# bioinfologics/w2rap-contigger

Measured on AMD Instinct MI355X. Metric: step2_k60_canonical_kmers_per_s, higher is better.
Workload: dtype u64

## Files before the change

### include/w2rap_step2.h

```cpp
#ifndef W2RAP_STEP2_H_
#define W2RAP_STEP2_H_

#include <stddef.h>
#include <stdint.h>

#ifdef __cplusplus
extern "C" {
#endif

#define W2RAP_STEP2_ABI_VERSION 3

enum {
    W2RAP_OK = 0,
    W2RAP_E_ARG = 1,
    W2RAP_E_NO_DEVICE = 2,
    W2RAP_E_HIP = 3,
    W2RAP_E_STATE = 4,
    W2RAP_E_LIMIT = 5,
    W2RAP_E_GRAPH = 6,
    W2RAP_E_HINT = 7,
    W2RAP_E_IO = 8
};

enum { W2RAP_MEM_HOST = 0, W2RAP_MEM_DEVICE = 1 };
// ... 124 lines not shown
int w2rap_step2_solid_buffers(w2rap_step2_ctx*, void** d_hi, void** d_lo, void** d_cc, uint64_t* n);
int w2rap_step2_set_solid(w2rap_step2_ctx*, const void* d_hi, const void* d_lo, const void* d_cc, uint64_t n,
                          uint64_t M, uint64_t D, const uint64_t* hist101);
int w2rap_step2_chunk_buffers(w2rap_step2_ctx*, void** d_chunk_start, void** d_chunk_count, uint64_t* n_chunks);
int w2rap_step2_set_solid_chunked(w2rap_step2_ctx*, const void* d_hi, const void* d_lo, const void* d_cc, uint64_t n,
                                  uint64_t M, uint64_t D, const uint64_t* hist101,
                                  const void* d_chunk_start, const void* d_chunk_count, uint64_t n_chunks);

int w2rap_step2_dict_begin(w2rap_step2_ctx*, uint64_t kmer_capacity, uint64_t chunk_capacity);
int w2rap_step2_dict_append(w2rap_step2_ctx*, const void* d_hi, const void* d_lo, const void* d_cc, uint64_t n,
                            const void* d_chunk_start, const void* d_chunk_count, uint64_t n_chunks);
int w2rap_step2_dict_append_slice(w2rap_step2_ctx*, const void* d_hi, const void* d_lo, const void* d_cc, uint64_t n,
                                  const void* d_chunk_start, const void* d_chunk_count, uint64_t n_chunks, uint64_t chunk_bias);
int w2rap_step2_dict_end(w2rap_step2_ctx*, uint64_t M, uint64_t D, const uint64_t* hist101);
int w2rap_step2_dict_abort(w2rap_step2_ctx*);

enum { W2RAP_X_DONE = 0, W2RAP_X_ALLTOALL = 1, W2RAP_X_ALLGATHER = 2, W2RAP_X_ALLGATHER_HOST = 3, W2RAP_X_ALLREDUCE_U8 = 4, W2RAP_X_ALLREDUCE_U32 = 5 };
typedef struct w2rap_xchg {
    int32_t  op;
    uint32_t elem_bytes;
    void*    send;
    uint64_t send_count[64];
} w2rap_xchg;
int w2rap_step2_shard_begin(w2rap_step2_ctx*, uint32_t rank, uint32_t world, const uint64_t* solid_per_rank ,
                            uint32_t n_buckets, uint32_t n_passes, uint64_t M, uint64_t D, const uint64_t* hist101,
                            const w2rap_edge_hint* hint );
int w2rap_step2_local_dict_slice(w2rap_step2_ctx*, uint64_t n_solid, uint64_t expected_total);
int w2rap_step2_shard_next(w2rap_step2_ctx*, w2rap_xchg* x);
int w2rap_step2_shard_recv(w2rap_step2_ctx*, const uint64_t* recv_count , uint32_t elem_bytes, void** d_recv);
int w2rap_step2_shard_host_words(w2rap_step2_ctx*, const uint64_t* words );
int w2rap_step2_shard_info(w2rap_step2_ctx*, uint64_t out[8]);
int w2rap_step2_selftest_prims(w2rap_step2_ctx*, uint64_t n, uint64_t seed, int key_bits);
int w2rap_step2_selftest_filter32(w2rap_step2_ctx*, uint64_t nbases, uint64_t seed, uint32_t w_lo_frac16, uint32_t w_hi_frac16);
uint64_t w2rap_step2_device_bytes(w2rap_step2_ctx*);
uint64_t w2rap_step2_device_peak_bytes(w2rap_step2_ctx*, int reset);

#ifdef __cplusplus
}
#endif
#endif
```

### w2rap_contigger_amd/csrc/common.h

```cpp
#pragma once
#include <hip/hip_runtime.h>
#include <stdint.h>

namespace w2 {

constexpr unsigned K = 60;
constexpr unsigned MMER_F = 15;
constexpr uint64_t M60 = (1ull << 60) - 1;
constexpr uint64_t EMPTY_HI = ~0ull;
constexpr uint32_t NONE32 = 0xFFFFFFFFu;

struct Kmer { uint64_t hi, lo; };

__host__ __device__ inline uint64_t rev2_64(uint64_t x) {
#if defined(__HIP_DEVICE_COMPILE__)
    x = __brevll(x);
#else
    x = ((x >> 1) & 0x5555555555555555ull) | ((x & 0x5555555555555555ull) << 1);
    x = ((x >> 2) & 0x3333333333333333ull) | ((x & 0x3333333333333333ull) << 2);
    x = ((x >> 4) & 0x0F0F0F0F0F0F0F0Full) | ((x & 0x0F0F0F0F0F0F0F0Full) << 4);
    x = __builtin_bswap64(x);
#endif
    return ((x >> 1) & 0x5555555555555555ull) | ((x & 0x5555555555555555ull) << 1);
}
// ... 130 lines not shown
    const unsigned long long x = w[v + RT_NODES - (o & 0xFFFu)];
    end = (Id)RankW<Id>::next(x);
    dist = end == v ? 0u : (uint32_t)RankW<Id>::dist(x) - (o >> 12);
}
template <class Id, unsigned U, class T>
__device__ inline void rank_of_staged(const uint32_t* __restrict__ own, const unsigned long long* __restrict__ w, const T* __restrict__ at_end,
                                      const uint64_t (&i)[U], Id (&end)[2 * U], uint32_t (&dist)[2 * U], T (&end_val)[2 * U]) {
    uint32_t o[2 * U]; unsigned long long x[2 * U];
#pragma unroll
    for (unsigned j = 0; j < U; ++j) { const uint2 t = *reinterpret_cast<const uint2*>(&own[2 * i[j]]); o[2 * j] = t.x; o[2 * j + 1] = t.y; }
#pragma unroll
    for (unsigned n = 0; n < 2 * U; ++n) {
        const uint64_t v = 2 * i[n / 2] + (n & 1);
        x[n] = w[o[n] == OWN_CIRCLE ? v : v + RT_NODES - (o[n] & 0xFFFu)];
    }
#pragma unroll
    for (unsigned n = 0; n < 2 * U; ++n) {
        const Id v = (Id)(2 * i[n / 2] + (n & 1));
        end[n] = o[n] == OWN_CIRCLE ? v : (Id)RankW<Id>::next(x[n]);
        dist[n] = end[n] == v ? 0u : (uint32_t)RankW<Id>::dist(x[n]) - (o[n] >> 12);
    }
#pragma unroll
    for (unsigned n = 0; n < 2 * U; ++n) end_val[n] = at_end[end[n]];
}
template <class Id>
__device__ inline uint32_t edge_of_end(const unsigned long long* __restrict__ w, Id t) {
    return (uint32_t)RankW<Id>::dist(w[t]) - 1u;
}

struct alignas(32) ObjRec { int32_t succ[4]; uint32_t eo_lo, eo_hi, elen, edge_rc ; };

constexpr unsigned FMER = 31;
constexpr unsigned FSPAN = K - FMER;
struct FmerKey { uint32_t word; uint64_t mask; };
__host__ __device__ inline FmerKey fmer_key(uint64_t x) {
    x &= (1ull << (2 * FMER)) - 1;
    const uint64_t rx = rev2_64(~x) >> (64 - 2 * FMER);
    uint32_t mu = 0xFFFFFFFFu;
#pragma unroll
    for (unsigned j = 0; j <= FMER - MMER_F; j += 4) {
        const uint32_t f = (uint32_t)(x >> (2 * j)) & 0x3FFFFFFFu, r = (uint32_t)(rx >> (2 * (FMER - MMER_F - j))) & 0x3FFFFFFFu;
        const uint32_t key = (f < r ? f : r) * 0x9E3779B1u;
        mu = key < mu ? key : mu;
    }
    uint32_t w = mu ^ (mu >> 15); w *= 0x85EBCA6Bu; w ^= w >> 13;
    const uint64_t h = (rx < x ? rx : x) * 0x9E3779B97F4A7C15ull;
    return FmerKey{w, (1ull << ((h >> 58) & 63)) | (1ull << ((h >> 40) & 63))};
}

#ifndef W2RAP_REC36
constexpr unsigned REC_DWORDS = 8;
constexpr unsigned REC_MAXK = 63;
constexpr unsigned REC_HB = 8;
#else
constexpr unsigned REC_DWORDS = 9;
constexpr unsigned REC_MAXK = 64;
constexpr unsigned REC_HB = 32;
#endif
constexpr unsigned REC_BYTES = 4 * REC_DWORDS;

__host__ __device__ inline void rec_build(const uint8_t* __restrict__ bases, uint64_t bases_bytes, uint64_t ro, uint32_t meta, uint32_t (&out)[REC_DWORDS]) {
    const unsigned p = meta & 0xFFFFu, nk = ((meta >> 16) & 63u) + 1u;
    const bool hasL = (meta >> 22) & 1u, hasR = (meta >> 23) & 1u;
    const unsigned q = p ? p - 1 : 0;
    const uint64_t byte0 = ro + ((2 * q) >> 3);
    const unsigned sh = (2 * q) & 7;
    uint64_t W[5];
#pragma unroll
    for (unsigned j = 0; j < 5; ++j) {
        const uint64_t a = byte0 + 8 * j;
        uint64_t w = 0;
        if (a + 8 <= bases_bytes) w = reinterpret_cast<const U64u*>(bases + a)->v;
        else for (unsigned t = 0; t < 8; ++t) if (a + t < bases_bytes) w |= (uint64_t)bases[a + t] << (8 * t);
        W[j] = w;
    }
    uint64_t O[4];
#pragma unroll
    for (unsigned j = 0; j < 4; ++j) O[j] = sh ? (W[j] >> sh) | (W[j + 1] << (64 - sh)) : W[j];
    if (!p) {
        O[3] = (O[3] << 2) | (O[2] >> 62); O[2] = (O[2] << 2) | (O[1] >> 62); O[1] = (O[1] << 2) | (O[0] >> 62); O[0] <<= 2;
// ... 207 lines not shown
```

### w2rap_contigger_amd/csrc/step2_graph.hip

```cpp
#include <algorithm>
#include <cstring>
#include <vector>
#include "ctx.h"

namespace w2 {

enum { GE_LOOKUP = 1, GE_OFFSET = 2, GE_HINT_MISS = 4, GE_HINT_DUP = 8, GE_ASSIGN = 16, GE_HINT_LEN = 32 };

template <class Id>
__device__ inline Kmer oriented(const uint64_t* shi, const uint64_t* slo, Id v) {
    Kmer k{shi[v >> 1], slo[v >> 1]};
    return (v & 1) ? kmer_rc(k) : k;
}

template <class Id>
__global__ void __launch_bounds__(256) k_links(uint64_t S, const uint64_t* __restrict__ shi, const uint64_t* __restrict__ slo,
                                                const uint8_t* __restrict__ sctx, Id* nbr_nxt0) {
    constexpr Id NONE = NodeId<Id>::NONE, PAL = NodeId<Id>::PAL;
    uint64_t i = (uint64_t)blockIdx.x * blockDim.x + threadIdx.x;
    if (i >= S) return;
    Kmer k{shi[i], slo[i]};
    Id n0 = NONE, n1 = NONE;
    if (!kmer_is_pal(k)) {
        const Id s = nbr_nxt0[2 * i], p = nbr_nxt0[2 * i + 1];
// ... 468 lines not shown
        } else dst[K - 1 + off[j]] = (uint8_t)kmer_last(k);
    }
}
template <class Id>
__global__ void __launch_bounds__(256) k_assign(uint64_t S, const uint64_t* __restrict__ shi, const uint64_t* __restrict__ slo,
                                                 const uint32_t* __restrict__ own, const unsigned long long* __restrict__ w,
                                                 const uint64_t* __restrict__ edge_off, KRec* __restrict__ srec,
                                                 uint8_t* __restrict__ codes, uint32_t* __restrict__ flags) {
    if (((uint64_t)blockIdx.x + 1) * (256 * RANK_U) <= S) assign_block<Id, true>(S, shi, slo, own, w, edge_off, srec, codes, flags);
    else assign_block<Id, false>(S, shi, slo, own, w, edge_off, srec, codes, flags);
}

__global__ void __launch_bounds__(256) k_pack_codes(uint64_t nbytes, uint64_t nbases, const uint8_t* __restrict__ codes, uint8_t* __restrict__ bits) {
    uint64_t i = (uint64_t)blockIdx.x * blockDim.x + threadIdx.x;
    if (i >= nbytes) return;
    unsigned v = 0;
#pragma unroll
    for (unsigned j = 0; j < 4; ++j) { uint64_t g = 4 * i + j; if (g < nbases) v |= (unsigned)(codes[g] & 3) << (2 * j); }
    bits[i] = (uint8_t)v;
}

__global__ void __launch_bounds__(256) k_filter32(uint64_t npos, const uint8_t* __restrict__ bits, unsigned long long* __restrict__ filter,
                                                   uint32_t fmask, uint32_t w_lo, uint32_t w_hi) {
    const uint64_t g = (uint64_t)blockIdx.x * blockDim.x + threadIdx.x;
    const unsigned lane = threadIdx.x & 63;
    uint32_t word = 0xFFFFFFFFu; unsigned long long mask = 0;
    if (g < npos) {
        const uint64_t b0 = g >> 2; const unsigned sh = 2 * (unsigned)(g & 3);
        uint64_t x = reinterpret_cast<const U64u*>(bits + b0)->v >> sh;
        if (sh) x |= (uint64_t)bits[b0 + 8] << (64 - sh);
        const FmerKey k = fmer_key(x);
        word = k.word & fmask; mask = k.mask;
    }
    const uint32_t prev = __shfl_up(word, 4);
    const bool head = g < npos && (lane < 4 || prev != word);
#pragma unroll
    for (unsigned d = 4; d < 64; d <<= 1) {
        const uint32_t ow = __shfl_down(word, d);
        const unsigned long long om = __shfl_down(mask, d);
        if (lane + d < 64 && ow == word) mask |= om;
    }
    if (head && word - w_lo < w_hi - w_lo) atomicOr(&filter[word - w_lo], mask);
}

__global__ void __launch_bounds__(256) k_index_tails(uint64_t E, const uint64_t* __restrict__ edge_off, const uint32_t* __restrict__ edge_nk,
                                                      uint32_t* __restrict__ bad) {
    const uint64_t e = (uint64_t)blockIdx.x * blockDim.x + threadIdx.x;
    if (e >= E) return;
    const uint64_t g1 = edge_off[e] + edge_nk[e] + (K - 1), g0 = g1 - (MMER - 1);
    for (uint64_t wd = g0 >> 5; wd <= (g1 - 1) >> 5; ++wd) {
        const uint64_t lo = wd << 5;
        const unsigned a = g0 > lo ? (unsigned)(g0 - lo) : 0u, b = g1 - lo < 32 ? (unsigned)(g1 - lo) : 32u;
        const uint32_t m = (b == 32 ? 0xFFFFFFFFu : (1u << b) - 1u) & ~((1u << a) - 1u);
        atomicOr(&bad[wd], m);
    }
}
constexpr unsigned IS = 2048, IT = IS - (WIN - 1);
constexpr unsigned IT_EDGES = IT / K + 3;
__global__ void __launch_bounds__(256) k_index_tile_edge(uint64_t E, const uint64_t* __restrict__ edge_off, uint32_t* __restrict__ tile_edge) {
    const uint64_t e = (uint64_t)blockIdx.x * blockDim.x + threadIdx.x;
    if (e >= E) return;
    const uint64_t a = edge_off[e], b = edge_off[e + 1];
    for (uint64_t t = (a + IT - 1) / IT; t * IT < b; ++t) tile_edge[t] = (uint32_t)e;
}
template <int MODE>
__global__ void __launch_bounds__(256) k_index_build(uint64_t nbases, const uint8_t* __restrict__ ebits, const uint32_t* __restrict__ bad, uint64_t E,
                                                      const uint64_t* __restrict__ edge_off, const uint32_t* __restrict__ tile_edge,
                                                      uint4* __restrict__ slots, uint64_t mask, unsigned long long* __restrict__ counter, uint64_t blk0) {
    constexpr bool WRITE = MODE != 0;
    constexpr unsigned NKEY = IS + (WIN - 1) + 3;
// ... 191 lines not shown
    uint64_t j = (uint64_t)blockIdx.x * blockDim.x + threadIdx.x;
    if (j >= n) return;
    uint32_t f = 0;
    if (j > 0) {
        uint32_t a = perm[j - 1], b = perm[j];
        const bool same_seq = ehi[a] == ehi[b] && elo[a] == elo[b];
        f = (ehash[a] != ehash[b] || !same_seq) ? 1u : 0u;
        if (ehash[a] == ehash[b] && !same_seq) *shared_hash = 1u;
    }
    flag[j] = f;
}
__global__ void __launch_bounds__(256) k_tie_sort_lo(uint64_t E, const uint64_t* __restrict__ shi, const uint64_t* __restrict__ lo, uint32_t* __restrict__ perm,
                                                      unsigned max_run, uint32_t* __restrict__ long_run ) {
    const uint64_t j = (uint64_t)blockIdx.x * blockDim.x + threadIdx.x;
    if (j >= E || (j > 0 && shi[j] == shi[j - 1])) return;
    uint64_t b = j + 1;
    while (b < E && shi[b] == shi[j]) ++b;
    if (b - j > max_run) { *long_run = 1u; return; }
    for (uint64_t i = j + 1; i < b; ++i) {
        const uint32_t x = perm[i]; const uint64_t lx = lo[x];
        uint64_t t = i;
        while (t > j && lo[perm[t - 1]] > lx) { perm[t] = perm[t - 1]; --t; }
        perm[t] = x;
    }
}
__global__ void __launch_bounds__(256) k_end_vertices(uint64_t n, const uint32_t* __restrict__ perm, const uint32_t* __restrict__ flag,
                                                       const uint64_t* __restrict__ excl, int32_t* __restrict__ left, int32_t* __restrict__ right) {
    uint64_t j = (uint64_t)blockIdx.x * blockDim.x + threadIdx.x;
    if (j >= n) return;
    int32_t vid = (int32_t)(excl[j] + flag[j]);
    uint32_t id = perm[j];
    if (id & 1) right[id >> 1] = vid; else left[id >> 1] = vid;
}
__global__ void __launch_bounds__(256) k_adj_keys(uint64_t NO, const int32_t* __restrict__ a, const int32_t* __restrict__ b,
                                                   uint64_t* __restrict__ keys, uint32_t* __restrict__ vals, uint32_t* __restrict__ deg) {
    uint64_t o = (uint64_t)blockIdx.x * blockDim.x + threadIdx.x;
    if (o >= NO) return;
    keys[o] = ((uint64_t)(uint32_t)a[o] << 32) | (uint32_t)b[o];
    vals[o] = (uint32_t)o;
    atomicAdd(&deg[a[o]], 1u);
}
__global__ void __launch_bounds__(256) k_adj_out(uint64_t NO, const uint32_t* __restrict__ vals, const int32_t* __restrict__ other,
                                                  int32_t* __restrict__ out_v, int32_t* __restrict__ out_e) {
    uint64_t j = (uint64_t)blockIdx.x * blockDim.x + threadIdx.x;
    if (j >= NO) return;
    uint32_t o = vals[j];
    out_e[j] = (int32_t)o; out_v[j] = other[o];
}

__device__ inline unsigned obj_base(const uint8_t* codes, uint64_t eoff, uint32_t len, bool rc, uint32_t t);
__global__ void __launch_bounds__(256) k_obj_table(uint64_t NO, const uint32_t* __restrict__ obj_edge, const uint32_t* __restrict__ edge_nk,
                                                    const uint64_t* __restrict__ edge_off, const uint8_t* __restrict__ codes,
                                                    const int32_t* __restrict__ right, const uint64_t* __restrict__ from_off,
                                                    const int32_t* __restrict__ from_e, ObjRec* __restrict__ tab) {
    const uint64_t o = (uint64_t)blockIdx.x * blockDim.x + threadIdx.x;
    if (o >= NO) return;
    const uint32_t oe = obj_edge[o], e = oe >> 1;
    const uint64_t eo = edge_off[e];
    ObjRec r;
    r.succ[0] = r.succ[1] = r.succ[2] = r.succ[3] = -1;
    r.eo_lo = (uint32_t)eo; r.eo_hi = (uint32_t)(eo >> 32); r.elen = edge_nk[e] + (K - 1); r.edge_rc = oe;
    const int32_t v = right[o];
    for (uint64_t k = from_off[v]; k < from_off[v + 1]; ++k) {
        const int32_t o2 = from_e[k];
        const uint32_t oe2 = obj_edge[o2], e2 = oe2 >> 1, len2 = edge_nk[e2] + (K - 1);
        const unsigned b = obj_base(codes, edge_off[e2], len2, oe2 & 1, K - 1);
        r.succ[b] = o2;
    }
    tab[o] = r;
}

// ... 570 lines not shown
    if (NE) {
        LAUNCH(c, "k_ends", k_ends, dim3(grid_for(NE)), dim3(256), 0, NO, c.d_obj_edge, c.d_edge_off, c.d_edge_nk, c.d_edge_codes, ehash, ehi, elo);
        bool by_bases = test_hook("W2RAP_TEST_ENDS_FULL_SORT");
        uint64_t nflag = 0;
        for (;;) {
            LAUNCH(c, "k_iota", k_iota, dim3(grid_for(NE)), dim3(256), 0, NE, eperm);
            if (by_bases) {
                LAUNCH(c, "k_gather_u64", k_gather_u64, dim3(grid_for(NE)), dim3(256), 0, NE, elo, eperm, ktmp);
                W2_TRY(sort_pairs_u64(c, ktmp, eperm, NE, 0, 58));
                LAUNCH(c, "k_gather_u64", k_gather_u64, dim3(grid_for(NE)), dim3(256), 0, NE, ehi, eperm, ktmp);
                W2_TRY(sort_pairs_u64(c, ktmp, eperm, NE, 0, 60));
            }
            LAUNCH(c, "k_gather_u64", k_gather_u64, dim3(grid_for(NE)), dim3(256), 0, NE, ehash, eperm, ktmp);
            W2_TRY(sort_pairs_u64(c, ktmp, eperm, NE, 0, 64));
            W2_HIP(hipMemsetAsync(d_flags + 3, 0, 4, st));
            LAUNCH(c, "k_end_flags", k_end_flags, dim3(grid_for(NE)), dim3(256), 0, NE, eperm, ehash, ehi, elo, eflag, d_flags + 3);
            W2_TRY(exclusive_scan_u32_to_u64(c, eflag, excl, NE));
            uint32_t shared_hash = 0;
            W2_HIP(hipMemcpyAsync(&nflag, excl + NE, 8, hipMemcpyDeviceToHost, st));
            W2_HIP(hipMemcpyAsync(&shared_hash, d_flags + 3, 4, hipMemcpyDeviceToHost, st));
            W2_HIP(hipStreamSynchronize(st));
            if (shared_hash && !by_bases) { by_bases = true; continue; }
            break;
        }
        c.NV = nflag + 1;
        LAUNCH(c, "k_end_vertices", k_end_vertices, dim3(grid_for(NE)), dim3(256), 0, NE, eperm, eflag, excl, c.d_left, c.d_right);
    }
    const uint64_t NV = c.NV;
    W2_ALLOC(c.d_from_off, uint64_t, NV + 1); W2_ALLOC(c.d_to_off, uint64_t, NV + 1);
    W2_ALLOC(c.d_from_v, int32_t, NO); W2_ALLOC(c.d_from_e, int32_t, NO);
    W2_ALLOC(c.d_to_v, int32_t, NO); W2_ALLOC(c.d_to_e, int32_t, NO);
    uint32_t* deg = nullptr; uint64_t* akeys = nullptr; uint32_t* avals = nullptr;
    W2_ALLOC(deg, uint32_t, NV); W2_ALLOC(akeys, uint64_t, NO); W2_ALLOC(avals, uint32_t, NO);
    for (int dir = 0; dir < 2; ++dir) {
        const int32_t* a = dir == 0 ? c.d_left : c.d_right;
        const int32_t* b = dir == 0 ? c.d_right : c.d_left;
        W2_HIP(hipMemsetAsync(deg, 0, (NV ? NV : 1) * 4, st));
        if (NO) {
            LAUNCH(c, "k_adj_keys", k_adj_keys, dim3(grid_for(NO)), dim3(256), 0, NO, a, b, akeys, avals, deg);
            W2_TRY(sort_pairs_u64(c, akeys, avals, NO, 0, 64));
            LAUNCH(c, "k_adj_out", k_adj_out, dim3(grid_for(NO)), dim3(256), 0, NO, avals, b, dir == 0 ? c.d_from_v : c.d_to_v,
                               dir == 0 ? c.d_from_e : c.d_to_e);
        }
        W2_TRY(exclusive_scan_u32_to_u64(c, deg, dir == 0 ? c.d_from_off : c.d_to_off, NV));
    }
    if (c.d_otab) { c.release(c.d_otab); c.d_otab = nullptr; }
    W2_ALLOC(c.d_otab, ObjRec, NO);
    if (NO) LAUNCH(c, "k_obj_table", k_obj_table, dim3(grid_for(NO)), dim3(256), 0, NO, c.d_obj_edge, c.d_edge_nk, c.d_edge_off, c.d_edge_codes,
                   c.d_right, c.d_from_off, c.d_from_e, c.d_otab);
    W2_HIP(hipStreamSynchronize(st));
    if (c.stream2) W2_HIP(hipStreamSynchronize(c.stream2));
    W2_HIP(hipGetLastError());
    for (void* p : {(void*)d_nobj, (void*)d_ooff, (void*)ehash, (void*)ehi, (void*)elo, (void*)ktmp, (void*)excl,
                    (void*)eperm, (void*)eflag, (void*)deg, (void*)akeys, (void*)avals, (void*)d_flags})
        c.release(p);
    c.graphed = true;
    return 0;
}

template <class Id>
static int phase_graph_t(Ctx& c, const w2rap_edge_hint* hint) {
    constexpr Id NONE = NodeId<Id>::NONE; (void)NONE;
    hipStream_t st = c.stream;
    const uint64_t S = c.S, N = 2 * S;
    const uint64_t mask = c.tcap - 1;
    uint32_t* d_flags = nullptr;
    W2_ALLOC(d_flags, uint32_t, 8);
    W2_HIP(hipMemsetAsync(d_flags, 0, 32, st));
    Id* nxt0 = reinterpret_cast<Id*>(c.d_nbr);
    unsigned long long* rankw = nullptr; uint32_t* own = nullptr;
    W2_ALLOC(rankw, unsigned long long, N); W2_ALLOC(own, uint32_t, N);
    uint8_t *cyc = nullptr, *mid = nullptr, *is_head = nullptr;
    W2_ALLOC(cyc, uint8_t, N); W2_ALLOC(mid, uint8_t, N);
// ... 77 lines not shown
    c.release(is_head); is_head = nullptr;
    uint32_t* d_elen = nullptr;
    W2_ALLOC(d_elen, uint32_t, E);
    W2_ALLOC(c.d_edge_off, uint64_t, E + 1);
    if (E) LAUNCH(c, "k_edge_len", k_edge_len, dim3(grid_for(E)), dim3(256), 0, E, c.d_edge_nk, d_elen);
    W2_TRY(exclusive_scan_u32_to_u64(c, d_elen, c.d_edge_off, E));
    W2_HIP(hipMemcpyAsync(&c.edge_bases, c.d_edge_off + E, 8, hipMemcpyDeviceToHost, st));
    W2_HIP(hipStreamSynchronize(st));
    W2_ALLOC(c.d_edge_codes, uint8_t, c.edge_bases + 64);
    {
        const char* iv = getenv("W2RAP_PATH_INDEX");
        c.use_index = iv && atoi(iv) != 0;
    }
    if (c.d_srec) { c.release(c.d_srec); c.d_srec = nullptr; }
    if (!c.use_index) W2_ALLOC(c.d_srec, KRec, S);
    if (S) LAUNCH(c, "k_assign", k_assign<Id>, dim3(grid_per_thread(S, RANK_U)), dim3(256), 0, S, c.d_shi, c.d_slo, own, rankw,
                              c.d_edge_off, c.d_srec, c.d_edge_codes, d_flags);
    W2_HIP(hipStreamSynchronize(st));
    c.release(rankw); c.release(own); rankw = nullptr; own = nullptr;
    for (void* p : {(void*)d_nheads, (void*)head_v, (void*)perm, (void*)edge_head, (void*)key_hi, (void*)key_lo, (void*)key_tmp, (void*)d_elen, (void*)d_flags})
        c.release(p);
    return graph_finish(c);
}

int phase_graph(Ctx& c, const w2rap_edge_hint* hint) {
    if (!c.counted) { c.err = "build_graph called before count_kmers"; return W2RAP_E_STATE; }
    if (!c.d_nbr && c.S) { c.err = "build_graph: the neighbour links of this count have been consumed; call count_kmers again"; return W2RAP_E_STATE; }
    c.graphed = false;
    return c.wide_ids ? phase_graph_t<uint64_t>(c, hint) : phase_graph_t<uint32_t>(c, hint);
}

}

extern "C" int w2rap_step2_selftest_filter32(w2rap_step2_ctx* h, uint64_t nbases, uint64_t seed, uint32_t w_lo_frac16, uint32_t w_hi_frac16) {
    using namespace w2;
    if (!h || nbases < FMER || nbases > (1ull << 33) || w_lo_frac16 > w_hi_frac16 || w_hi_frac16 > 16) return -1;
    Ctx& c = h->c;
    if (hipSetDevice(c.device) != hipSuccess) return -1;
    const uint64_t nby = (nbases + 3) / 4;
    std::vector<uint8_t> hb(nby + 16, 0);
    uint64_t x = seed * 0x9E3779B97F4A7C15ull + 1;
    for (uint64_t g = 0; g < nbases; ++g) {
        x ^= x << 13; x ^= x >> 7; x ^= x << 17;
        hb[g >> 2] |= (uint8_t)(((x >> 33) & 3) << (2 * (g & 3)));
    }
    const uint64_t fw = filter32_words_for(nbases), lo = fw * w_lo_frac16 / 16, hi = fw * w_hi_frac16 / 16, npos = nbases - (FMER - 1);
    std::vector<unsigned long long> want(hi - lo + 1, 0), got(hi - lo + 1);
    for (uint64_t g = 0; g < npos; ++g) {
        const uint64_t b0 = g >> 2; const unsigned sh = 2 * (unsigned)(g & 3);
        uint64_t v; std::memcpy(&v, &hb[b0], 8);
        v >>= sh;
        if (sh) v |= (uint64_t)hb[b0 + 8] << (64 - sh);
        const FmerKey k = fmer_key(v);
        const uint64_t word = k.word & (uint32_t)(fw - 1);
        if (word >= lo && word < hi) want[word - lo] |= k.mask;
    }
    uint8_t* d_bits = c.alloc<uint8_t>(nby + 16, false);
    unsigned long long* d_out = c.alloc<unsigned long long>(hi - lo + 1, false);
    if (!d_bits || !d_out) return -1;
    int bad = 0;
    if (hipMemcpyAsync(d_bits, hb.data(), nby + 16, hipMemcpyHostToDevice, c.stream) != hipSuccess ||
        filter32_build(c, c.stream, d_bits, nbases, fw, lo, hi, d_out, hi - lo + 1) ||
        hipMemcpyAsync(got.data(), d_out, (hi - lo + 1) * 8, hipMemcpyDeviceToHost, c.stream) != hipSuccess ||
        hipStreamSynchronize(c.stream) != hipSuccess) bad = -1;
    for (uint64_t i = 0; i < hi - lo && !bad; ++i) if (got[i] != want[i]) bad = 1;
    if (!bad && got[hi - lo] != 0) bad = 2;
    c.release(d_bits); c.release(d_out);
    return bad;
}
```

### w2rap_contigger_amd/csrc/step2_path.hip

```cpp
#include <algorithm>
#include <cstdlib>
#include <type_traits>
#include "ctx.h"

namespace w2 {

#ifdef W2RAP_IDX_STATS
#define SITE_STAT(k) do { const unsigned long long am_ = __ballot(1); if ((threadIdx.x & 63) == (unsigned)__builtin_ctzll(am_)) { atomicAdd(&g_site_stats[2 * (k)], (unsigned long long)__builtin_popcountll(am_)); atomicAdd(&g_site_stats[2 * (k) + 1], 1ull); } } while (0)
static __device__ unsigned long long g_site_stats[8];
#else
#define SITE_STAT(k) ((void)0)
#endif
constexpr unsigned PCS = 256;
constexpr unsigned LP = 2;
constexpr unsigned PL = 4;
constexpr unsigned PATH_THREADS = 256;
constexpr uint32_t LONG_READ = 1024;
constexpr uint64_t SCRATCH_CAP = 16ull << 30;
constexpr uint64_t LONG_SCRATCH = 2ull << 30;
#ifndef W2RAP_PATH_TICKETS
#define W2RAP_PATH_TICKETS 1
#endif
constexpr uint32_t PATH_TICKETS = W2RAP_PATH_TICKETS;
struct PathArgs {
// ... 306 lines not shown
        const uint64_t bo = A.boff[live ? r : (LISTED ? r : r0)];
        bool deferred = false;
        uint32_t my_off = 0;
        if (STAGED) {
            const uint64_t b_lo = A.boff[r0], b_hi = A.boff[r0 + nr], a0 = b_lo & ~3ull;
            const uint32_t nbytes = (uint32_t)(b_hi - a0), nfull = nbytes >> 2;
            const uint32_t* src = reinterpret_cast<const uint32_t*>(A.bases + a0);
            for (uint32_t i = tid; i < nfull; i += PATH_THREADS) s_rd[i] = src[i];
            if (tid < 4) s_rd[nfull + 1 + tid] = 0;
            if (tid == 0) {
                uint32_t v = 0;
                for (uint32_t t2 = 0; t2 < (nbytes & 3); ++t2) v |= (uint32_t)A.bases[a0 + 4ull * nfull + t2] << (8 * t2);
                s_rd[nfull] = v;
            }
            my_off = (uint32_t)(bo - a0);
            __syncthreads();
        }
        uint32_t plen = 0, lo = A.pmid, hi = A.pmid;
        int32_t offset = 0;
        if (live) {
#ifdef W2RAP_IDX_STATS
            const unsigned long long ts0 = __builtin_amdgcn_s_memtime();
#endif
            const uint8_t* rb = A.bases + bo;
            const uint8_t* q = A.quals + A.qoff[r];
            const uint32_t L = A.len[r];
            uint32_t np = 0;
            typename std::conditional<STAGED, RdLds, RdGlb>::type rd;
            if constexpr (STAGED) { rd.w = s_rd; rd.off = my_off; } else { rd.rb = rb; rd.nby = (L + 3) >> 2; }
            if (L < K) { setp(0, make_gap(L)); np = 1; }
            else {
                uint32_t p = 0;
                const uint32_t end = L - K + 1;
                auto mer32_at = [&](uint32_t tt) -> FmerKey { return fmer_key(rd.bits64(tt)); };
                auto f32_absent = [&](const FmerKey& k, unsigned long long w) -> bool { return (w & k.mask) != k.mask; };
                const uint32_t last = L - K, tmax = L - FMER;
                auto probe3 = [&](uint32_t cur0, uint32_t e) -> uint32_t {
                    const uint32_t qmax = e < last ? e : last;
                    auto target = [&](uint32_t c_) -> uint32_t { uint32_t tt = c_ + FSPAN < e ? c_ + FSPAN : e; return tt > tmax ? tmax : tt; };
                    uint32_t cur = cur0;
                    const bool v0 = cur <= qmax; const uint32_t t0 = target(cur), q0 = t0 < last ? t0 : last; if (v0) cur = q0 + 1;
                    const bool v1 = v0 && cur <= qmax; const uint32_t t1 = target(cur), q1 = t1 < last ? t1 : last; if (v1) cur = q1 + 1;
                    const bool v2 = v1 && cur <= qmax; const uint32_t t2 = target(cur), q2 = t2 < last ? t2 : last;
                    FmerKey k0{0, 0}, k1{0, 0}, k2{0, 0}; unsigned long long w0 = 0, w1 = 0, w2 = 0;
                    if (v0) { k0 = mer32_at(t0); w0 = A.filter32[k0.word & A.f32mask]; }
                    if (v1) { k1 = mer32_at(t1); w1 = A.filter32[k1.word & A.f32mask]; }
                    if (v2) { k2 = mer32_at(t2); w2 = A.filter32[k2.word & A.f32mask]; }
                    const bool a0 = v0 && f32_absent(k0, w0), a1 = a0 && v1 && f32_absent(k1, w1), a2 = a1 && v2 && f32_absent(k2, w2);
                    return a2 ? q2 + 1 - cur0 : a1 ? q1 + 1 - cur0 : a0 ? q0 + 1 - cur0 : 0u;
                };
                bool mism = false;
                uint32_t pv_e = 0, pv_elen = 0, pv_i = 0, pv_j = 0; uint64_t pv_eo = 0; bool pv_rc = false;
                bool at_end = false;
                int32_t pv_obj = 0;
                while (p != end) {
                    if (!LISTED && A.part_budget && np >= A.part_budget) { deferred = true; break; }
                    bool hit = false; IdxHit ih{};
                    auto lookup = [&](uint32_t pp) -> bool { return dict_lookup<INDEX>(A, rd, pp, ih); };
                    uint32_t gapLen = 0;
                    bool probed = false;
                    const bool after_mism = mism;
                    if (mism && A.filter32) { gapLen = probe3(p, p + (K - 1)); p += gapLen; probed = gapLen != 0; }
                    mism = false;
                    bool diag_hit = false; uint32_t dg_off = 0;
                    bool ask_dict = !gapLen;
                    if (at_end) {
                        const unsigned nb_ = (unsigned)(rd.bits64(p + (K - 1)) & 3u);
// ... 175 lines not shown
            const unsigned want = (unsigned)__builtin_popcountll(free_m);
            const int leader = __builtin_ctzll(free_m);
            unsigned long long base = 0;
            if ((int)lane == leader) base = atomicAdd(&A.stripes[(size_t)stripe * STRIPE_PAD], (unsigned long long)want);
            base = __shfl(base, leader);
            const uint64_t s_lo = (uint64_t)stripe * per_stripe, s_hi = s_lo + per_stripe < n_all ? s_lo + per_stripe : n_all;
            const uint64_t idx = s_lo + base + (unsigned)__builtin_popcountll(free_m & ((1ull << lane) - 1));
            if (!has && !ready && idx < s_hi) {
                r = A.r_first + idx;
                const uint64_t bo = A.boff[r];
                L = A.len[r];
                const uint32_t nby = (L + 3) >> 2;
                for (uint32_t o = 0; o < A.slot_dwords * 4; o += 16) {
                    uint4 v = make_uint4(0, 0, 0, 0);
                    if (o < nby + 8) {
                        if (bo + o + 16 <= A.bases_bytes) { const U128u w = *reinterpret_cast<const U128u*>(A.bases + bo + o); v = make_uint4((uint32_t)w.a, (uint32_t)(w.a >> 32), (uint32_t)w.b, (uint32_t)(w.b >> 32)); }
                        else {
                            uint32_t t4[4] = {0, 0, 0, 0};
                            for (uint32_t t2 = 0; t2 < 16 && bo + o + t2 < A.bases_bytes; ++t2) t4[t2 >> 2] |= (uint32_t)A.bases[bo + o + t2] << (8 * (t2 & 3));
                            v = make_uint4(t4[0], t4[1], t4[2], t4[3]);
                        }
                    }
                    *reinterpret_cast<uint4*>(slot + (o >> 2)) = v;
                }
                has = true; deferred = false; np = 0; p = 0; mism = false; at_end = false;
                if (L < K) { setp(0, make_gap(L)); np = 1; end = 0; }
                else end = L - K + 1;
            }
            if (s_lo + base + want >= s_hi) { ++stripes_done; stripe = (stripe + 1) % NSTR; }
        }
        if (has && p != end) {
            if (A.part_budget && np >= A.part_budget) { deferred = true; p = end; }
            else {
                auto mer32_at = [&](uint32_t tt) -> FmerKey { return fmer_key(rd.bits64(tt)); };
                auto f32_absent = [&](const FmerKey& k, unsigned long long w) -> bool { return (w & k.mask) != k.mask; };
                const uint32_t last = L - K, tmax = L - FMER;
                auto probe3 = [&](uint32_t cur0, uint32_t e) -> uint32_t {
                    const uint32_t qmax = e < last ? e : last;
                    auto target = [&](uint32_t c_) -> uint32_t { uint32_t tt = c_ + FSPAN < e ? c_ + FSPAN : e; return tt > tmax ? tmax : tt; };
                    uint32_t cur = cur0;
                    const bool v0 = cur <= qmax; const uint32_t t0 = target(cur), q0 = t0 < last ? t0 : last; if (v0) cur = q0 + 1;
                    const bool v1 = v0 && cur <= qmax; const uint32_t t1 = target(cur), q1 = t1 < last ? t1 : last; if (v1) cur = q1 + 1;
                    const bool v2 = v1 && cur <= qmax; const uint32_t t2 = target(cur), q2 = t2 < last ? t2 : last;
                    FmerKey k0{0, 0}, k1{0, 0}, k2{0, 0}; unsigned long long w0 = 0, w1 = 0, w2 = 0;
                    if (v0) { k0 = mer32_at(t0); w0 = A.filter32[k0.word & A.f32mask]; }
                    if (v1) { k1 = mer32_at(t1); w1 = A.filter32[k1.word & A.f32mask]; }
                    if (v2) { k2 = mer32_at(t2); w2 = A.filter32[k2.word & A.f32mask]; }
                    const bool a0 = v0 && f32_absent(k0, w0), a1 = a0 && v1 && f32_absent(k1, w1), a2 = a1 && v2 && f32_absent(k2, w2);
                    return a2 ? q2 + 1 - cur0 : a1 ? q1 + 1 - cur0 : a0 ? q0 + 1 - cur0 : 0u;
                };
                bool hit = false; IdxHit ih{};
                auto lookup = [&](uint32_t pp) -> bool { return dict_lookup<INDEX>(A, rd, pp, ih); };
                uint32_t gapLen = 0;
                bool probed = false;
                const bool after_mism = mism;
                if (mism && A.filter32) { gapLen = probe3(p, p + (K - 1)); p += gapLen; probed = gapLen != 0; }
                mism = false;
                bool diag_hit = false; uint32_t dg_off = 0;
                bool ask_dict = !gapLen;
                if (at_end) {
                    const unsigned nb_ = (unsigned)(rd.bits64(p + (K - 1)) & 3u);
                    const int32_t o2 = A.otab[pv_obj].succ[nb_];
                    if (o2 >= 0) {
                        const ObjRec r2 = A.otab[o2];
                        diag_hit = true; dg_off = 0; ask_dict = false;
                        pv_e = r2.edge_rc >> 1; pv_rc = r2.edge_rc & 1u; pv_elen = r2.elen; pv_eo = (uint64_t)r2.eo_lo | ((uint64_t)r2.eo_hi << 32);
                    }
// ... 617 lines not shown
```

Measured before the change: 44.91 billion.

## Sample filter minimizers at stride two and narrow adjacency sort keys

The 31-mer filter key now takes the minimizer over window offsets at stride 2 instead of 4. This gives denser minimizer sampling, so more equal filter words are shared between neighbouring positions and the path-stage filter probes should give fewer false hits, at the cost of more hashing work per key and scheduling barriers in the path kernels. The gather shuffle distance follows the new stride. Separately, adjacency sort keys pack vertex ids into only as many bits as needed, so the radix sort runs over fewer key bits. A periodic-sequence self-test for the filter is added.

```diff
diff --git a/include/w2rap_step2.h b/include/w2rap_step2.h
--- a/include/w2rap_step2.h
+++ b/include/w2rap_step2.h
@@ -180,6 +180,7 @@
 int w2rap_step2_shard_info(w2rap_step2_ctx*, uint64_t out[8]);
 int w2rap_step2_selftest_prims(w2rap_step2_ctx*, uint64_t n, uint64_t seed, int key_bits);
 int w2rap_step2_selftest_filter32(w2rap_step2_ctx*, uint64_t nbases, uint64_t seed, uint32_t w_lo_frac16, uint32_t w_hi_frac16);
+int w2rap_step2_selftest_filter32_periodic(w2rap_step2_ctx*, uint64_t nbases, uint32_t period, uint64_t seed, uint32_t w_lo_frac16, uint32_t w_hi_frac16);
 uint64_t w2rap_step2_device_bytes(w2rap_step2_ctx*);
 uint64_t w2rap_step2_device_peak_bytes(w2rap_step2_ctx*, int reset);
 
diff --git a/w2rap_contigger_amd/csrc/common.h b/w2rap_contigger_amd/csrc/common.h
--- a/w2rap_contigger_amd/csrc/common.h
+++ b/w2rap_contigger_amd/csrc/common.h
@@ -186,20 +186,34 @@
 
 constexpr unsigned FMER = 31;
 constexpr unsigned FSPAN = K - FMER;
+#ifndef W2RAP_FMER_STRIDE
+#define W2RAP_FMER_STRIDE 2
+#endif
+constexpr unsigned FMER_STRIDE = W2RAP_FMER_STRIDE;
+static_assert(FMER_STRIDE >= 1 && (FMER - MMER_F) % FMER_STRIDE == 0, "the window offsets must map onto themselves under j <-> 16 - j");
 struct FmerKey { uint32_t word; uint64_t mask; };
+template <unsigned STRIDE = FMER_STRIDE, bool FENCED = false>
 __host__ __device__ inline FmerKey fmer_key(uint64_t x) {
+    static_assert(STRIDE >= 1 && (FMER - MMER_F) % STRIDE == 0, "stride must divide 16");
     x &= (1ull << (2 * FMER)) - 1;
     const uint64_t rx = rev2_64(~x) >> (64 - 2 * FMER);
     uint32_t mu = 0xFFFFFFFFu;
-#pragma unroll
-    for (unsigned j = 0; j <= FMER - MMER_F; j += 4) {
+#if defined(__HIP_DEVICE_COMPILE__)
+    if (FENCED) __builtin_amdgcn_sched_barrier(0);
+#endif
+#pragma unroll
+    for (unsigned j = 0; j <= FMER - MMER_F; j += STRIDE) {
         const uint32_t f = (uint32_t)(x >> (2 * j)) & 0x3FFFFFFFu, r = (uint32_t)(rx >> (2 * (FMER - MMER_F - j))) & 0x3FFFFFFFu;
         const uint32_t key = (f < r ? f : r) * 0x9E3779B1u;
         mu = key < mu ? key : mu;
     }
     uint32_t w = mu ^ (mu >> 15); w *= 0x85EBCA6Bu; w ^= w >> 13;
     const uint64_t h = (rx < x ? rx : x) * 0x9E3779B97F4A7C15ull;
-    return FmerKey{w, (1ull << ((h >> 58) & 63)) | (1ull << ((h >> 40) & 63))};
+    const FmerKey k{w, (1ull << ((h >> 58) & 63)) | (1ull << ((h >> 40) & 63))};
+#if defined(__HIP_DEVICE_COMPILE__)
+    if (FENCED) __builtin_amdgcn_sched_barrier(0);
+#endif
+    return k;
 }
 
 #ifndef W2RAP_REC36
diff --git a/w2rap_contigger_amd/csrc/step2_graph.hip b/w2rap_contigger_amd/csrc/step2_graph.hip
--- a/w2rap_contigger_amd/csrc/step2_graph.hip
+++ b/w2rap_contigger_amd/csrc/step2_graph.hip
@@ -524,10 +524,12 @@
         const FmerKey k = fmer_key(x);
         word = k.word & fmask; mask = k.mask;
     }
-    const uint32_t prev = __shfl_up(word, 4);
-    const bool head = g < npos && (lane < 4 || prev != word);
-#pragma unroll
-    for (unsigned d = 4; d < 64; d <<= 1) {
+    constexpr unsigned D = FMER_STRIDE;
+    static_assert(D <= 32 && (D & (D - 1)) == 0, "the gather doubles its distance up to 32");
+    const uint32_t prev = __shfl_up(word, D);
+    const bool head = g < npos && (lane < D || prev != word);
+#pragma unroll
+    for (unsigned d = D; d < 64; d <<= 1) {
         const uint32_t ow = __shfl_down(word, d);
         const unsigned long long om = __shfl_down(mask, d);
         if (lane + d < 64 && ow == word) mask |= om;
@@ -785,11 +787,11 @@
     uint32_t id = perm[j];
     if (id & 1) right[id >> 1] = vid; else left[id >> 1] = vid;
 }
-__global__ void __launch_bounds__(256) k_adj_keys(uint64_t NO, const int32_t* __restrict__ a, const int32_t* __restrict__ b,
+__global__ void __launch_bounds__(256) k_adj_keys(uint64_t NO, const int32_t* __restrict__ a, const int32_t* __restrict__ b, unsigned vbits,
                                                    uint64_t* __restrict__ keys, uint32_t* __restrict__ vals, uint32_t* __restrict__ deg) {
     uint64_t o = (uint64_t)blockIdx.x * blockDim.x + threadIdx.x;
     if (o >= NO) return;
-    keys[o] = ((uint64_t)(uint32_t)a[o] << 32) | (uint32_t)b[o];
+    keys[o] = ((uint64_t)(uint32_t)a[o] << vbits) | (uint32_t)b[o];
     vals[o] = (uint32_t)o;
     atomicAdd(&deg[a[o]], 1u);
 }
@@ -1426,13 +1428,15 @@
     W2_ALLOC(c.d_to_v, int32_t, NO); W2_ALLOC(c.d_to_e, int32_t, NO);
     uint32_t* deg = nullptr; uint64_t* akeys = nullptr; uint32_t* avals = nullptr;
     W2_ALLOC(deg, uint32_t, NV); W2_ALLOC(akeys, uint64_t, NO); W2_ALLOC(avals, uint32_t, NO);
+    unsigned vbits = 1;
+    while (vbits < 32 && ((NV ? NV - 1 : 0) >> vbits)) ++vbits;
     for (int dir = 0; dir < 2; ++dir) {
         const int32_t* a = dir == 0 ? c.d_left : c.d_right;
         const int32_t* b = dir == 0 ? c.d_right : c.d_left;
         W2_HIP(hipMemsetAsync(deg, 0, (NV ? NV : 1) * 4, st));
         if (NO) {
-            LAUNCH(c, "k_adj_keys", k_adj_keys, dim3(grid_for(NO)), dim3(256), 0, NO, a, b, akeys, avals, deg);
-            W2_TRY(sort_pairs_u64(c, akeys, avals, NO, 0, 64));
+            LAUNCH(c, "k_adj_keys", k_adj_keys, dim3(grid_for(NO)), dim3(256), 0, NO, a, b, vbits, akeys, avals, deg);
+            W2_TRY(sort_pairs_u64(c, akeys, avals, NO, 0, (int)(2 * vbits)));
             LAUNCH(c, "k_adj_out", k_adj_out, dim3(grid_for(NO)), dim3(256), 0, NO, avals, b, dir == 0 ? c.d_from_v : c.d_to_v,
                                dir == 0 ? c.d_from_e : c.d_to_e);
         }
@@ -1576,7 +1580,7 @@
 
 }
 
-extern "C" int w2rap_step2_selftest_filter32(w2rap_step2_ctx* h, uint64_t nbases, uint64_t seed, uint32_t w_lo_frac16, uint32_t w_hi_frac16) {
+static int selftest_filter32_stream(w2rap_step2_ctx* h, uint64_t nbases, uint64_t seed, uint32_t period, uint32_t w_lo_frac16, uint32_t w_hi_frac16) {
     using namespace w2;
     if (!h || nbases < FMER || nbases > (1ull << 33) || w_lo_frac16 > w_hi_frac16 || w_hi_frac16 > 16) return -1;
     Ctx& c = h->c;
@@ -1585,8 +1589,10 @@
     std::vector<uint8_t> hb(nby + 16, 0);
     uint64_t x = seed * 0x9E3779B97F4A7C15ull + 1;
     for (uint64_t g = 0; g < nbases; ++g) {
-        x ^= x << 13; x ^= x >> 7; x ^= x << 17;
-        hb[g >> 2] |= (uint8_t)(((x >> 33) & 3) << (2 * (g & 3)));
+        unsigned b;
+        if (period && g >= period) b = (hb[(g - period) >> 2] >> (2 * ((g - period) & 3))) & 3u;
+        else { x ^= x << 13; x ^= x >> 7; x ^= x << 17; b = (unsigned)((x >> 33) & 3); }
+        hb[g >> 2] |= (uint8_t)(b << (2 * (g & 3)));
     }
     const uint64_t fw = filter32_words_for(nbases), lo = fw * w_lo_frac16 / 16, hi = fw * w_hi_frac16 / 16, npos = nbases - (FMER - 1);
     std::vector<unsigned long long> want(hi - lo + 1, 0), got(hi - lo + 1);
@@ -1612,3 +1618,11 @@
     c.release(d_bits); c.release(d_out);
     return bad;
 }
+extern "C" int w2rap_step2_selftest_filter32(w2rap_step2_ctx* h, uint64_t nbases, uint64_t seed, uint32_t w_lo_frac16, uint32_t w_hi_frac16) {
+    return selftest_filter32_stream(h, nbases, seed, 0, w_lo_frac16, w_hi_frac16);
+}
+extern "C" int w2rap_step2_selftest_filter32_periodic(w2rap_step2_ctx* h, uint64_t nbases, uint32_t period, uint64_t seed, uint32_t w_lo_frac16,
+                                                      uint32_t w_hi_frac16) {
+    if (!period) return -1;
+    return selftest_filter32_stream(h, nbases, seed, period, w_lo_frac16, w_hi_frac16);
+}
diff --git a/w2rap_contigger_amd/csrc/step2_path.hip b/w2rap_contigger_amd/csrc/step2_path.hip
--- a/w2rap_contigger_amd/csrc/step2_path.hip
+++ b/w2rap_contigger_amd/csrc/step2_path.hip
@@ -362,7 +362,7 @@
             else {
                 uint32_t p = 0;
                 const uint32_t end = L - K + 1;
-                auto mer32_at = [&](uint32_t tt) -> FmerKey { return fmer_key(rd.bits64(tt)); };
+                auto mer32_at = [&](uint32_t tt) -> FmerKey { return fmer_key<FMER_STRIDE, (FMER_STRIDE < 4)>(rd.bits64(tt)); };
                 auto f32_absent = [&](const FmerKey& k, unsigned long long w) -> bool { return (w & k.mask) != k.mask; };
                 const uint32_t last = L - K, tmax = L - FMER;
                 auto probe3 = [&](uint32_t cur0, uint32_t e) -> uint32_t {
@@ -604,7 +604,7 @@
         if (has && p != end) {
             if (A.part_budget && np >= A.part_budget) { deferred = true; p = end; }
             else {
-                auto mer32_at = [&](uint32_t tt) -> FmerKey { return fmer_key(rd.bits64(tt)); };
+                auto mer32_at = [&](uint32_t tt) -> FmerKey { return fmer_key<FMER_STRIDE, (FMER_STRIDE < 4)>(rd.bits64(tt)); };
                 auto f32_absent = [&](const FmerKey& k, unsigned long long w) -> bool { return (w & k.mask) != k.mask; };
                 const uint32_t last = L - K, tmax = L - FMER;
                 auto probe3 = [&](uint32_t cur0, uint32_t e) -> uint32_t {
```

New measurement: 45.49 billion, median of 6. 1.3% higher.
